# cvlab-stonybrook/s-volsdf

Hardware: AMD Instinct MI355X
Metric: rendered rays/sec (1024-ray batch, 128 samples) (higher is better)
Workload: dtype f32 (every product, forward and backward, as three fp16 MFMA products of two-piece fp16 operands with f32 accumulate; activation blocks hold both pieces: float32 accuracy class); 1 GPU; configs[1]: VolOpt.train_step (forward + MVS prior lookup + loss + backward + clip/guard/Adam), train mode, fast=1: 1024 rays/GPU x 128 coarse + 98 composited samples + 2048 eikonal points, 8x256 SDF MLP + 4x256 radiance MLP; mode=train, mlp_precision=fp16x2, launch=eager launches, rays_per_gpu=1024, rays_total=1024

## Files before the change

s-volsdf_amd/csrc/svs_wgrad.hip:

```cpp
#include "svs_common.h"
#include "svs_mlp_layout.h"
#include "svs_ticket.h"
#include <cstdlib>

namespace svs {
namespace wgrad {

struct Pair {
  const float* a;
  const float* b;
  size_t stride_a, stride_b;
};

struct Args {
  Pair p[2];
  int n_pairs;
  int n_tiles;
  int n_valid_points;
  const float* b_extra;
  size_t stride_extra;
  float* dW;
  int ldw;
  float* db;
  det::Ticket ticket;
};

struct Staging {
  f32x4 a[8], b[8], x;
};

template <int NTB>
__global__ __launch_bounds__(256, 1) void wgrad_kernel(Args a) {
  constexpr int PA = 260, PB = NTB == 9 ? 292 : 260;
  constexpr int BUF = 32 * (PA + PB);
  extern __shared__ __attribute__((aligned(16))) float smem[];
  const int tid = threadIdx.x, wave = tid >> 6, lane = tid & 63;
  const int half = lane >> 5, col = lane & 31;
  f32x16 acc[2][NTB];
#pragma unroll
  for (int o = 0; o < 2; ++o)
#pragma unroll
    for (int i = 0; i < NTB; ++i) acc[o][i] = (f32x16)(0.0f);
  float bias_acc = 0.0f;

  const int my_tiles = a.n_tiles > (int)blockIdx.x ? (a.n_tiles - 1 - (int)blockIdx.x) / (int)gridDim.x + 1 : 0;
  const int n_items = my_tiles * a.n_pairs;
  Staging st;
  int st_live = 32;

  auto issue = [&](int item) {
    const int t = blockIdx.x + (item / a.n_pairs) * gridDim.x, pi = item % a.n_pairs;
    const Pair& p = a.p[pi];
    const f32x4* ga = reinterpret_cast<const f32x4*>(p.a + (size_t)t * p.stride_a);
    const f32x4* gb = reinterpret_cast<const f32x4*>(p.b + (size_t)t * p.stride_b);
#pragma unroll
    for (int k = 0; k < 8; ++k) { st.a[k] = ga[k * 256 + tid]; st.b[k] = gb[k * 256 + tid]; }
    if (NTB == 9) {
      st.x = (a.b_extra && pi == 0) ? reinterpret_cast<const f32x4*>(a.b_extra + (size_t)t * a.stride_extra)[tid]
                                    : (f32x4)(0.0f);
    }
    st_live = a.n_valid_points - t * 32;
  };
  auto commit = [&](int buf) {
    float* la = smem + buf * BUF;
    float* lb = la + 32 * PA;
    if (st_live < 32) {
#pragma unroll
      for (int k = 0; k < 8; ++k) if ((tid & 31) >= st_live) st.a[k] = (f32x4)(0.0f);
    }
#pragma unroll
    for (int k = 0; k < 8; ++k) {
      const int q = k * 256 + tid, i4 = q >> 6, ln = q & 63;
      const int feat = 32 * (i4 >> 2) + 8 * (i4 & 3) + 4 * (ln >> 5), pt = ln & 31;
      *reinterpret_cast<f32x4*>(la + pt * PA + feat) = st.a[k];
      *reinterpret_cast<f32x4*>(lb + pt * PB + feat) = st.b[k];
    }
    if (NTB == 9) {
      const int i4 = tid >> 6, ln = tid & 63;
      *reinterpret_cast<f32x4*>(lb + (ln & 31) * PB + 256 + 8 * i4 + 4 * (ln >> 5)) = st.x;
    }
  };

  if (n_items > 0) { issue(0); commit(0); }
  __syncthreads();
  for (int item = 0; item < n_items; ++item) {
    const int buf = item & 1;
    const bool more = item + 1 < n_items;
    if (more) issue(item + 1);
    const float* la = smem + buf * BUF;
    const float* lb = la + 32 * PA;
    if (a.db && (item % a.n_pairs) == 0) {
      float s = 0.0f;
#pragma unroll 8
      for (int q = 0; q < 32; ++q) s += la[q * PA + tid];
      bias_acc += s;
    }
#pragma unroll 4
    for (int s = 0; s < 16; ++s) {
      const int pt = 2 * s + half;
      const float a0 = la[pt * PA + 32 * (2 * wave) + col];
      const float a1 = la[pt * PA + 32 * (2 * wave + 1) + col];
#pragma unroll
      for (int i = 0; i < NTB; ++i) {
        const float b = lb[pt * PB + 32 * i + col];
        acc[0][i] = __builtin_amdgcn_mfma_f32_32x32x2f32(a0, b, acc[0][i], 0, 0, 0);
        acc[1][i] = __builtin_amdgcn_mfma_f32_32x32x2f32(a1, b, acc[1][i], 0, 0, 0);
      }
    }
    if (more) commit(buf ^ 1);
    __syncthreads();
  }
  det::wait_turn(a.ticket, blockIdx.x);
#pragma unroll
  for (int o = 0; o < 2; ++o)
#pragma unroll
    for (int i = 0; i < NTB; ++i)
#pragma unroll
      for (int r = 0; r < 16; ++r) {
        const int row = 32 * (2 * wave + o) + rho(r) + 4 * half;
        const int c = 32 * i + col;
        if (c < a.ldw) atomicAdd(&a.dW[(size_t)row * a.ldw + c], acc[o][i][r]);
      }
  if (a.db) atomicAdd(&a.db[tid], bias_acc);
  det::pass_turn(a.ticket, blockIdx.x);
}


namespace h2 {

typedef _Float16 f16x8 __attribute__((ext_vector_type(8)));
typedef _Float16 f16x4 __attribute__((ext_vector_type(4)));
typedef _Float16 f16x2 __attribute__((ext_vector_type(2)));
typedef short s16x4 __attribute__((__vector_size__(4 * sizeof(short))));
#define SVS_LDS(T, ptr) ((__attribute__((address_space(3))) T*)(ptr))

constexpr int kPlane = 16384;
constexpr int kExtraPiece = 32 * 64;
constexpr int kNarrowImg = 8192;
constexpr int kRecBytes = 8 * 256;
constexpr int kFactorBytes = 8 * 64;
template <bool GP>
struct Ring {
  static constexpr int kPlanes = GP ? 2 : 1;
  static constexpr int kSlot = 2 * kPlanes * kPlane;
  static constexpr int kB = kPlanes * kPlane;
  static constexpr int kRing = GP ? 2 : 4;
  static constexpr int kAhead = kRing - 1;
  static constexpr int kSlotAll = kSlot + kRecBytes + kFactorBytes;
  static constexpr int kLdsBytes = kRing * kSlotAll;
};

struct Frag { s16x4 lo, hi; };
__device__ __forceinline__ void tr_issue(Frag& v, unsigned a0, unsigned a1) {
  asm volatile("ds_read_b64_tr_b16 %0, %1" : "=v"(v.lo) : "v"(a0));
  asm volatile("ds_read_b64_tr_b16 %0, %1" : "=v"(v.hi) : "v"(a1));
}
__device__ __forceinline__ f16x8 frag_of(const Frag& v) { return __builtin_bit_cast(f16x8, v); }
__device__ __forceinline__ void lds_read128(f32x4& v, unsigned a) { asm volatile("ds_read_b128 %0, %1" : "=v"(v) : "v"(a)); }
__device__ __forceinline__ void lds_read32(float& v, unsigned a) { asm volatile("ds_read_b32 %0, %1" : "=v"(v) : "v"(a)); }
__device__ __forceinline__ void lds_wait() {
  asm volatile("s_waitcnt lgkmcnt(0)" ::: "memory");
  __builtin_amdgcn_sched_barrier(0);
}
__device__ __forceinline__ unsigned lds_addr(const void* p) {
  return (unsigned)(unsigned long long)SVS_LDS(const void, p);
}

__device__ __forceinline__ void scale_from_absmax(const float* absmax, float& s, float& inv_s) {
  s = 1.0f; inv_s = 1.0f;
  if (!absmax) return;
  int e = (int)((__float_as_uint(*absmax) >> 23) & 0xff);
  e = e < 16 ? 16 : (e > 250 ? 250 : e);
  s = __uint_as_float((unsigned)(268 - e) << 23);
  inv_s = __uint_as_float((unsigned)(e - 14) << 23);
}

struct Job {
  Pair p[2];
  const float* rec[2];
  int n_pairs;
  int n_tiles;
  int n_valid_points;
  int b_tiles;
  int col0;
  float* dW;
  int ldw;
  float* db;
  const float* absmax;
  int wg_begin, wg_count;
  det::Ticket ticket;
};
constexpr int kMaxJobs = 20;
struct MultiArgs { Job job[kMaxJobs]; int n_jobs; int touch; int reverse; };
static_assert(sizeof(MultiArgs) <= 4096, "kernel arguments");

constexpr int kThreadsW = 512;

typedef const __attribute__((address_space(1))) void* gvoid;

template <bool GP>
__global__ __launch_bounds__(kThreadsW, 1) void wgrad_h2_multi_kernel(MultiArgs ma) {
  typedef Ring<GP> R;
  constexpr int kSlot = R::kSlot, kSlotAll = R::kSlotAll, kRing = R::kRing, kAhead = R::kAhead, kB = R::kB;
  extern __shared__ __attribute__((aligned(16))) unsigned char smem_h2[];
  int jj = 0;
  for (int q = 1; q < ma.n_jobs; ++q) if ((int)blockIdx.x >= ma.job[q].wg_begin) jj = q;
  const Job& a = ma.job[jj];
  const int wg = (int)blockIdx.x - a.wg_begin, nwg = a.wg_count;
  const int tid = threadIdx.x, lane = tid & 63;
  const int wave = __builtin_amdgcn_readfirstlane(tid >> 6);
  const bool narrow = a.b_tiles == 1;
  float s_grad, inv_s;
  scale_from_absmax(a.absmax, s_grad, inv_s);

  f32x16 acc[8];
#pragma unroll
  for (int i = 0; i < 8; ++i) acc[i] = (f32x16)(0.0f);
  float bsum = 0.0f;

  unsigned char* ring = smem_h2;

  const int rq = (lane & 15) >> 2, rp = lane & 3, rg = (lane >> 4) & 1, rh = lane >> 5;
  const int rd0 = 1024 * rg + 256 * rh + 128 * rg + 64 * (rp & 1) + 16 * rq + 8 * (rp >> 1);
  const int a_rd = 2048 * wave + rd0;
  const int rx0 = 64 * (8 * rh + rq) + 32 * rg + 8 * rp, rx1 = rx0 + 64 * 4;
  const int wp = lane & 31, whf = lane >> 5;
  const int wxoff = 64 * wp + 16 * (wave & 3) + 8 * whf;

  const bool two_pairs = a.n_pairs == 2;
  const int my_tiles = a.n_tiles > wg ? (a.n_tiles - 1 - wg) / nwg + 1 : 0;
  const int n_items = two_pairs ? 2 * my_tiles : my_tiles;
  const int n_valid = a.n_valid_points;
  const bool has_db = a.db != nullptr;
  const bool rev = ma.reverse != 0;
  const float* const pa0 = a.p[0].a; const float* const pb0 = a.p[0].b;
  const float* const pa1 = a.p[1].a; const float* const pb1 = a.p[1].b;
  const size_t sa0 = a.p[0].stride_a, sb0 = a.p[0].stride_b, sa1 = a.p[1].stride_a, sb1 = a.p[1].stride_b;
  const float* const rec0 = a.rec[0]; const float* const rec1 = a.rec[1];
  const bool has_scale = a.absmax != nullptr;
  auto tile_of = [&](int item) {
    const int k = two_pairs ? item >> 1 : item;
    return rev ? wg + (my_tiles - 1 - k) * nwg : wg + k * nwg;
  };

  auto issue = [&](int item) {
    const int t = tile_of(item), pi = two_pairs ? item & 1 : 0;
    const float* pa = (pi ? pa1 : pa0) + (size_t)t * (pi ? sa1 : sa0);
    const float* pb = (pi ? pb1 : pb0) + (size_t)t * (pi ? sb1 : sb0);
    unsigned char* slot = ring + (item % kRing) * kSlotAll;
#pragma unroll
    for (int j = 0; j < 2 * R::kPlanes; ++j) {
      const int piece = wave + 8 * j;
      __builtin_amdgcn_global_load_lds((gvoid)(reinterpret_cast<const f32x4*>(pa) + piece * 64 + lane),
                                       SVS_LDS(void, slot + piece * 1024), 16, 0, 0);
      if (!narrow)
        __builtin_amdgcn_global_load_lds((gvoid)(reinterpret_cast<const f32x4*>(pb) + piece * 64 + lane),
                                         SVS_LDS(void, slot + kB + piece * 1024), 16, 0, 0);
    }
    if (narrow)
      __builtin_amdgcn_global_load_lds((gvoid)(reinterpret_cast<const f32x4*>(pb) + (wave & 3) * 64 + lane),
                                       SVS_LDS(void, slot + kB + (wave & 3) * 1024), 16, 0, 0);
    if (has_scale)
      __builtin_amdgcn_global_load_lds((gvoid)((pi ? rec1 : rec0) + (size_t)t * 64 + lane),
                                       SVS_LDS(void, slot + kSlot + wave * 256), 4, 0, 0);
  };
  unsigned sink = 0;
  auto touch = [&](int item) {
    const int t = tile_of(item), pi = two_pairs ? item & 1 : 0;
    const Pair& p = a.p[pi];
    constexpr int kLines = R::kPlanes * (kPlane / 128);
    const int nb = narrow ? 32 : kLines;
    const float* q = tid < kLines ? p.a + (size_t)t * p.stride_a + tid * 32
                                  : p.b + (size_t)t * p.stride_b + (tid - kLines) * 32;
    if (tid < kLines + nb) asm volatile("global_load_dword %0, %1, off" : "+v"(sink) : "v"(q) : "memory");
  };
  const int ops = (narrow ? 2 * R::kPlanes + 1 : 4 * R::kPlanes) + (has_scale ? 1 : 0);

  auto stage_factors = [&](int item) {
    unsigned char* slot = ring + (item % kRing) * kSlotAll;
    const int t = tile_of(item);
    const int live = n_valid - t * 32;
    float f = 1.0f;
    if (has_scale) {
      float rec;
      lds_read32(rec, lds_addr(slot + kSlot + wave * 256 + 4 * wp));
      lds_wait();
      const unsigned eb = (__float_as_uint(rec) >> 23) & 0xff;
      if (eb >= 20 && eb <= 240) f = __builtin_fminf(s_grad * __uint_as_float((254u << 23) - __float_as_uint(rec)), 32768.0f);
    }
    if (wp >= live) f = 0.0f;
    if (lane < 32) asm volatile("ds_write_b16 %0, %1" :: "v"(lds_addr(slot + kSlot + kRecBytes + wave * 64 + 2 * lane)), "v"((_Float16)f) : "memory");
  };
  auto stage_narrow = [&](int item) {
    unsigned char* slot = ring + (item % kRing) * kSlotAll;
    if (tid < 256) {
      f32x4 v;
      lds_read128(v, lds_addr(slot + kB + tid * 16));
      lds_wait();
      f16x4 hi, mid;
#pragma unroll
      for (int j = 0; j < 4; ++j) {
        const _Float16 h = (_Float16)v[j];
        hi[j] = h;
        mid[j] = (_Float16)(v[j] - (float)h);
      }
      *SVS_LDS(f16x4, slot + kB + kNarrowImg + wxoff) = hi;
      *SVS_LDS(f16x4, slot + kB + kNarrowImg + kExtraPiece + wxoff) = mid;
    }
  };

  const f16x2 one2 = {(_Float16)1.0f, (_Float16)1.0f};

  for (int i0 = 0; i0 < kAhead && i0 < n_items; ++i0) issue(i0);
  const bool touching = GP && ma.touch;
  bool touched = false;
  if (touching && kAhead < n_items) { touch(kAhead); touched = true; }
  auto pre_stage = [&](int it) {
    const int left = n_items - 1 - it;
    const int later = (left < kAhead - 1 ? left : kAhead - 1) * ops;
    if (later == 10) asm volatile("s_waitcnt vmcnt(10)" ::: "memory");
    else if (later == 8) asm volatile("s_waitcnt vmcnt(8)" ::: "memory");
    else if (later == 6) asm volatile("s_waitcnt vmcnt(6)" ::: "memory");
    else if (later == 5) asm volatile("s_waitcnt vmcnt(5)" ::: "memory");
    else if (later == 4) asm volatile("s_waitcnt vmcnt(4)" ::: "memory");
    else if (later == 3) asm volatile("s_waitcnt vmcnt(3)" ::: "memory");
    else if (touched) asm volatile("s_waitcnt vmcnt(1)" ::: "memory");
    else asm volatile("s_waitcnt vmcnt(0)" ::: "memory");
    stage_factors(it);
  };
  for (int item = 0; item < n_items; ++item) {
    const int pi = two_pairs ? item & 1 : 0;
    const bool p0 = pi == 0;
    pre_stage(item);
    asm volatile("s_waitcnt lgkmcnt(0)\n\ts_barrier" ::: "memory");
    if (narrow) {
      stage_narrow(item);
      asm volatile("s_waitcnt lgkmcnt(0)\n\ts_barrier" ::: "memory");
    }
    auto issue_next = [&]() {
      if (item + kAhead < n_items) issue(item + kAhead);
      touched = false;
      if (touching && item + kAhead + 1 < n_items) { touch(item + kAhead + 1); touched = true; }
    };
    const unsigned la = lds_addr(ring + (item % kRing) * kSlotAll);
    const unsigned lb = la + kB;
    const unsigned ftab = la + kSlot + kRecBytes + wave * 64;
    const unsigned nimg = lb + kNarrowImg;
    const bool want_bias = has_db && p0;
    const bool two = narrow;
    Frag fa2[2], fam2[2];
    f32x4 fraw2[2];
#pragma unroll
    for (int ks = 0; ks < 2; ++ks) {
      tr_issue(fa2[ks], la + 512 * ks + a_rd, la + 512 * ks + (a_rd ^ 128));
      if (GP) tr_issue(fam2[ks], la + kPlane + 512 * ks + a_rd, la + kPlane + 512 * ks + (a_rd ^ 128));
      lds_read128(fraw2[ks], ftab + 32 * ks + 16 * rh);
    }
    issue_next();
    lds_wait();
#pragma unroll
    for (int ks = 0; ks < 2; ++ks) {
      const f16x8 ah = frag_of(fa2[ks]) * __builtin_bit_cast(f16x8, fraw2[ks]);
      const f16x8 am = GP ? frag_of(fam2[ks]) * __builtin_bit_cast(f16x8, fraw2[ks]) : ah;
      if (want_bias) {
#pragma unroll
        for (int j = 0; j < 4; ++j) {
          const f16x2 h2v = {ah[2 * j], ah[2 * j + 1]};
          bsum = __builtin_amdgcn_fdot2(h2v, one2, bsum, false);
          if (GP) {
            const f16x2 m2v = {am[2 * j], am[2 * j + 1]};
            bsum = __builtin_amdgcn_fdot2(m2v, one2, bsum, false);
          }
        }
      }
#pragma unroll
      for (int i = 0; i < 8; ++i) {
        if (i > 0 && narrow) break;
        Frag fh, fm;
        if (!narrow) {
          const unsigned rd = lb + 2048 * i + 512 * ks + rd0;
          tr_issue(fh, rd, rd ^ 128);
          if (GP) tr_issue(fm, rd + kPlane, (rd ^ 128) + kPlane);
        } else {
          tr_issue(fh, nimg + ks * 1024 + rx0, nimg + ks * 1024 + rx1);
          tr_issue(fm, nimg + kExtraPiece + ks * 1024 + rx0, nimg + kExtraPiece + ks * 1024 + rx1);
        }
        lds_wait();
        if (two || GP) acc[i] = __builtin_amdgcn_mfma_f32_32x32x16_f16(ah, frag_of(fm), acc[i], 0, 0, 0);
        if (GP) acc[i] = __builtin_amdgcn_mfma_f32_32x32x16_f16(am, frag_of(fh), acc[i], 0, 0, 0);
        acc[i] = __builtin_amdgcn_mfma_f32_32x32x16_f16(ah, frag_of(fh), acc[i], 0, 0, 0);
      }
    }
  }
  asm volatile("s_waitcnt vmcnt(0)" :: "v"(sink) : "memory");
  const int half = lane >> 5, col = lane & 31;
  det::wait_turn(a.ticket, wg);
#pragma unroll
  for (int i = 0; i < 8; ++i) {
    if (i > 0 && narrow) break;
#pragma unroll
    for (int r = 0; r < 16; ++r) {
      const int row = 32 * wave + rho(r) + 4 * half;
      const int c = a.col0 + 32 * i + col;
      if (c < a.ldw) atomicAdd(&a.dW[(size_t)row * a.ldw + c], acc[i][r] * inv_s);
    }
  }
  if (a.db) {
    bsum += __shfl_xor(bsum, 32);
    if (half == 0) atomicAdd(&a.db[32 * wave + col], bsum * inv_s);
  }
  det::pass_turn(a.ticket, wg);
}

}

}
}

using namespace svs;
using namespace svs::wgrad;
namespace h2 = svs::wgrad::h2;

extern "C" {

struct svs_wgrad_job {
  const float *a0, *b0; long long sa0, sb0;
  const float *a1, *b1; long long sa1, sb1;
  const float* b_extra; long long s_extra;
  int n_points, ldw;
  float *dW, *db;
  const float* absmax;
  const float *rec0, *rec1;
};

int svs_wgrad_multi(const svs_wgrad_job* jobs, int n_jobs, int precision, void* hip_stream) {
  if (!jobs || n_jobs < 1) { set_error("svs_wgrad_multi: no jobs"); return SVS_EINVAL; }
  int n_expanded = 0;
  for (int j = 0; j < n_jobs; ++j) n_expanded += jobs[j].b_extra ? 2 : 1;
  if (n_expanded > h2::kMaxJobs) { set_error("svs_wgrad_multi: at most %d jobs (b_extra counts twice)", h2::kMaxJobs); return SVS_EINVAL; }
  for (int j = 0; j < n_jobs; ++j) {
    const svs_wgrad_job& q = jobs[j];
    if (!q.a0 || !q.b0 || !q.dW || q.n_points <= 0 || q.ldw < 256 || q.ldw > 288 || (q.b_extra && q.ldw < 288) || (q.a1 && !q.b1)) {
      set_error("svs_wgrad_multi: bad argument in job %d", j); return SVS_EINVAL;
    }
    if (mlp::is_h2(precision) && q.absmax && (!q.rec0 || (q.a1 && !q.rec1))) {
      set_error("svs_wgrad_multi: job %d has absmax but no scale records", j); return SVS_EINVAL;
    }
  }
  hipStream_t s = (hipStream_t)hip_stream;
  if (mlp::is_h2(precision)) {
    const bool gp = precision == mlp::kFmtF16x2;
    h2::MultiArgs ma;
    int n = 0;
    long long work[h2::kMaxJobs], total = 0;
    for (int j = 0; j < n_jobs; ++j) {
      const svs_wgrad_job& q = jobs[j];
      h2::Job& J = ma.job[n];
      J.p[0] = Pair{q.a0, q.b0, (size_t)q.sa0, (size_t)q.sb0};
      J.rec[0] = q.rec0; J.rec[1] = q.rec1;
      J.n_pairs = 1;
      if (q.a1) { J.p[1] = Pair{q.a1, q.b1, (size_t)q.sa1, (size_t)q.sb1}; J.n_pairs = 2; }
      else { J.p[1] = J.p[0]; J.rec[1] = J.rec[0]; }
      J.n_tiles = (q.n_points + 31) / 32; J.n_valid_points = q.n_points;
      J.b_tiles = 8; J.col0 = 0; J.dW = q.dW; J.ldw = q.ldw; J.db = q.db; J.absmax = q.absmax;
      work[n] = (long long)J.n_tiles * J.n_pairs * 10;
      total += work[n++];
      if (q.b_extra) {
        h2::Job& X = ma.job[n];
        X = J;
        X.p[0].b = q.b_extra; X.p[0].stride_b = (size_t)q.s_extra; X.n_pairs = 1;
        X.b_tiles = 1; X.col0 = 256; X.db = nullptr;
        work[n] = (long long)X.n_tiles * 6;
        total += work[n++];
      }
    }
    ma.n_jobs = n;
    static const int touch_env = [] { const char* e = getenv("SVS_WGRAD_TOUCH"); return e ? atoi(e) : 0; }();
    ma.touch = touch_env;
    static const int reverse_env = [] { const char* e = getenv("SVS_WGRAD_REVERSE"); return e ? atoi(e) : 0; }();
    ma.reverse = reverse_env;
    (void)total;
    const int n_wg_total = 256;
    int count[h2::kMaxJobs];
    int used = 0;
    for (int j = 0; j < n; ++j) { count[j] = 1; ++used; }
    while (used < n_wg_total) {
      int best = -1;
      double load = 0.0;
      for (int j = 0; j < n; ++j) {
        if (count[j] >= ma.job[j].n_tiles) continue;
        const double l = (double)work[j] / count[j];
        if (l > load) { load = l; best = j; }
      }
      if (best < 0) break;
      ++count[best]; ++used;
    }
    int begin = 0;
    for (int j = 0; j < n; ++j) {
      ma.job[j].wg_begin = begin; ma.job[j].wg_count = count[j];
      begin += count[j];
      ma.job[j].ticket = det::Ticket{nullptr, 0u, 0u};
    }
    if (deterministic()) {
      int owner[h2::kMaxJobs], n_owner = 0;
      for (int j = 0; j < n; ++j) {
        owner[j] = -1;
        for (int k = 0; k < j; ++k)
          if (ma.job[k].dW == ma.job[j].dW && ma.job[k].col0 == ma.job[j].col0) { owner[j] = owner[k]; break; }
        if (owner[j] < 0) owner[j] = n_owner++;
      }
      unsigned* turn = det::take_slots((unsigned)n_owner);
      if (!turn) { set_error("svs_wgrad_multi: no turn counters (deterministic mode)"); return SVS_EINVAL; }
      unsigned total[h2::kMaxJobs] = {0};
      for (int j = 0; j < n; ++j) { ma.job[j].ticket.turn = turn + owner[j]; ma.job[j].ticket.first = total[owner[j]]; total[owner[j]] += (unsigned)count[j]; }
      for (int j = 0; j < n; ++j) ma.job[j].ticket.total = total[owner[j]];
    }
    static hipError_t e = hipFuncSetAttribute(reinterpret_cast<const void*>(h2::wgrad_h2_multi_kernel<false>),
                                              hipFuncAttributeMaxDynamicSharedMemorySize, h2::Ring<false>::kLdsBytes);
    static hipError_t ep = hipFuncSetAttribute(reinterpret_cast<const void*>(h2::wgrad_h2_multi_kernel<true>),
                                               hipFuncAttributeMaxDynamicSharedMemorySize, h2::Ring<true>::kLdsBytes);
    if (e != hipSuccess || ep != hipSuccess) {
      set_error("svs_wgrad_multi: hipFuncSetAttribute: %s", hipGetErrorString(e != hipSuccess ? e : ep)); return (int)(e != hipSuccess ? e : ep);
    }
    if (gp) h2::wgrad_h2_multi_kernel<true><<<begin, h2::kThreadsW, h2::Ring<true>::kLdsBytes, s>>>(ma);
    else h2::wgrad_h2_multi_kernel<false><<<begin, h2::kThreadsW, h2::Ring<false>::kLdsBytes, s>>>(ma);
    return check_launch("svs_wgrad_multi");
  }
  if (precision != mlp::kFmtF32) { set_error("svs_wgrad_multi: unknown precision %d", precision); return SVS_EINVAL; }
  for (int j = 0; j < n_jobs; ++j) {
    const svs_wgrad_job& q = jobs[j];
    Args a;
    a.p[0] = Pair{q.a0, q.b0, (size_t)q.sa0, (size_t)q.sb0};
    a.n_pairs = 1;
    if (q.a1) { a.p[1] = Pair{q.a1, q.b1, (size_t)q.sa1, (size_t)q.sb1}; a.n_pairs = 2; }
    a.n_tiles = (q.n_points + 31) / 32;
    a.n_valid_points = q.n_points;
    a.b_extra = q.b_extra; a.stride_extra = (size_t)q.s_extra;
    a.dW = q.dW; a.ldw = q.ldw; a.db = q.db;
    const int grid = a.n_tiles < 256 ? a.n_tiles : 256;
    a.ticket = det::Ticket{det::take_slots(1), 0u, (unsigned)grid};
    if (q.b_extra) {
      constexpr int lds = 2 * 32 * (260 + 292) * 4;
      static hipError_t e9 = hipFuncSetAttribute(reinterpret_cast<const void*>(wgrad_kernel<9>),
                                                 hipFuncAttributeMaxDynamicSharedMemorySize, lds);
      if (e9 != hipSuccess) { set_error("svs_wgrad_multi: hipFuncSetAttribute: %s", hipGetErrorString(e9)); return (int)e9; }
      wgrad_kernel<9><<<grid, 256, lds, s>>>(a);
    } else {
      constexpr int lds = 2 * 32 * (260 + 260) * 4;
      static hipError_t e8 = hipFuncSetAttribute(reinterpret_cast<const void*>(wgrad_kernel<8>),
                                                 hipFuncAttributeMaxDynamicSharedMemorySize, lds);
      if (e8 != hipSuccess) { set_error("svs_wgrad_multi: hipFuncSetAttribute: %s", hipGetErrorString(e8)); return (int)e8; }
      wgrad_kernel<8><<<grid, 256, lds, s>>>(a);
    }
    if (int rc = check_launch("svs_wgrad_multi")) return rc;
  }
  return SVS_OK;
}

int svs_wgrad(const float* a0, const float* b0, long long sa0, long long sb0, const float* a1, const float* b1,
              long long sa1, long long sb1, const float* b_extra, long long s_extra, int n_points, int precision,
              const float* absmax, const float* rec0, const float* rec1, float* dW, int ldw, float* db, void* hip_stream) {
  svs_wgrad_job q{a0, b0, sa0, sb0, a1, b1, sa1, sb1, b_extra, s_extra, n_points, ldw, dW, db, absmax, rec0, rec1};
  return svs_wgrad_multi(&q, 1, precision, hip_stream);
}

}
```

Before: 290,600 rays/s.

## Fold extra-input weight-gradient columns into the main wgrad job

```diff
diff --git a/s-volsdf_amd/csrc/svs_wgrad.hip b/s-volsdf_amd/csrc/svs_wgrad.hip
--- a/s-volsdf_amd/csrc/svs_wgrad.hip
+++ b/s-volsdf_amd/csrc/svs_wgrad.hip
@@ -136,7 +136,7 @@
 
 constexpr int kPlane = 16384;
 constexpr int kExtraPiece = 32 * 64;
-constexpr int kNarrowImg = 8192;
+constexpr int kExtraBytes = 4096;
 constexpr int kRecBytes = 8 * 256;
 constexpr int kFactorBytes = 8 * 64;
 template <bool GP>
@@ -147,8 +147,11 @@
   static constexpr int kRing = GP ? 2 : 4;
   static constexpr int kAhead = kRing - 1;
   static constexpr int kSlotAll = kSlot + kRecBytes + kFactorBytes;
-  static constexpr int kLdsBytes = kRing * kSlotAll;
+  static constexpr int kXRaw = kRing * kSlotAll;
+  static constexpr int kXImg = kXRaw + kAhead * kExtraBytes;
+  static constexpr int kLdsBytes = kXImg + 2 * kExtraBytes;
 };
+static_assert(Ring<true>::kLdsBytes <= 160 * 1024 && Ring<false>::kLdsBytes <= 160 * 1024, "LDS of a CU");
 
 struct Frag { s16x4 lo, hi; };
 __device__ __forceinline__ void tr_issue(Frag& v, unsigned a0, unsigned a1) {
@@ -181,8 +184,8 @@
   int n_pairs;
   int n_tiles;
   int n_valid_points;
-  int b_tiles;
-  int col0;
+  const float* x;
+  size_t stride_x;
   float* dW;
   int ldw;
   float* db;
@@ -209,13 +212,12 @@
   const int wg = (int)blockIdx.x - a.wg_begin, nwg = a.wg_count;
   const int tid = threadIdx.x, lane = tid & 63;
   const int wave = __builtin_amdgcn_readfirstlane(tid >> 6);
-  const bool narrow = a.b_tiles == 1;
   float s_grad, inv_s;
   scale_from_absmax(a.absmax, s_grad, inv_s);
 
-  f32x16 acc[8];
-#pragma unroll
-  for (int i = 0; i < 8; ++i) acc[i] = (f32x16)(0.0f);
+  f32x16 acc[9];
+#pragma unroll
+  for (int i = 0; i < 9; ++i) acc[i] = (f32x16)(0.0f);
   float bsum = 0.0f;
 
   unsigned char* ring = smem_h2;
@@ -238,6 +240,11 @@
   const size_t sa0 = a.p[0].stride_a, sb0 = a.p[0].stride_b, sa1 = a.p[1].stride_a, sb1 = a.p[1].stride_b;
   const float* const rec0 = a.rec[0]; const float* const rec1 = a.rec[1];
   const bool has_scale = a.absmax != nullptr;
+  const float* const px = a.x;
+  const size_t sx = a.stride_x;
+  const bool has_x = px != nullptr;
+  const bool x_wave = has_x && wave < 4;
+  const unsigned xraw = lds_addr(ring + R::kXRaw), ximg = lds_addr(ring + R::kXImg);
   auto tile_of = [&](int item) {
     const int k = two_pairs ? item >> 1 : item;
     return rev ? wg + (my_tiles - 1 - k) * nwg : wg + k * nwg;
@@ -253,13 +260,12 @@
       const int piece = wave + 8 * j;
       __builtin_amdgcn_global_load_lds((gvoid)(reinterpret_cast<const f32x4*>(pa) + piece * 64 + lane),
                                        SVS_LDS(void, slot + piece * 1024), 16, 0, 0);
-      if (!narrow)
-        __builtin_amdgcn_global_load_lds((gvoid)(reinterpret_cast<const f32x4*>(pb) + piece * 64 + lane),
-                                         SVS_LDS(void, slot + kB + piece * 1024), 16, 0, 0);
-    }
-    if (narrow)
-      __builtin_amdgcn_global_load_lds((gvoid)(reinterpret_cast<const f32x4*>(pb) + (wave & 3) * 64 + lane),
-                                       SVS_LDS(void, slot + kB + (wave & 3) * 1024), 16, 0, 0);
+      __builtin_amdgcn_global_load_lds((gvoid)(reinterpret_cast<const f32x4*>(pb) + piece * 64 + lane),
+                                       SVS_LDS(void, slot + kB + piece * 1024), 16, 0, 0);
+    }
+    if (x_wave)
+      __builtin_amdgcn_global_load_lds((gvoid)(reinterpret_cast<const f32x4*>(px + (size_t)t * sx) + wave * 64 + lane),
+                                       SVS_LDS(void, ring + R::kXRaw + (item % kAhead) * kExtraBytes + wave * 1024), 16, 0, 0);
     if (has_scale)
       __builtin_amdgcn_global_load_lds((gvoid)((pi ? rec1 : rec0) + (size_t)t * 64 + lane),
                                        SVS_LDS(void, slot + kSlot + wave * 256), 4, 0, 0);
@@ -269,12 +275,11 @@
     const int t = tile_of(item), pi = two_pairs ? item & 1 : 0;
     const Pair& p = a.p[pi];
     constexpr int kLines = R::kPlanes * (kPlane / 128);
-    const int nb = narrow ? 32 : kLines;
     const float* q = tid < kLines ? p.a + (size_t)t * p.stride_a + tid * 32
                                   : p.b + (size_t)t * p.stride_b + (tid - kLines) * 32;
-    if (tid < kLines + nb) asm volatile("global_load_dword %0, %1, off" : "+v"(sink) : "v"(q) : "memory");
-  };
-  const int ops = (narrow ? 2 * R::kPlanes + 1 : 4 * R::kPlanes) + (has_scale ? 1 : 0);
+    if (tid < 2 * kLines) asm volatile("global_load_dword %0, %1, off" : "+v"(sink) : "v"(q) : "memory");
+  };
+  const int ops = 4 * R::kPlanes + (has_scale ? 1 : 0) + (x_wave ? 1 : 0);
 
   auto stage_factors = [&](int item) {
     unsigned char* slot = ring + (item % kRing) * kSlotAll;
@@ -291,22 +296,20 @@
     if (wp >= live) f = 0.0f;
     if (lane < 32) asm volatile("ds_write_b16 %0, %1" :: "v"(lds_addr(slot + kSlot + kRecBytes + wave * 64 + 2 * lane)), "v"((_Float16)f) : "memory");
   };
-  auto stage_narrow = [&](int item) {
-    unsigned char* slot = ring + (item % kRing) * kSlotAll;
-    if (tid < 256) {
-      f32x4 v;
-      lds_read128(v, lds_addr(slot + kB + tid * 16));
-      lds_wait();
-      f16x4 hi, mid;
-#pragma unroll
-      for (int j = 0; j < 4; ++j) {
-        const _Float16 h = (_Float16)v[j];
-        hi[j] = h;
-        mid[j] = (_Float16)(v[j] - (float)h);
-      }
-      *SVS_LDS(f16x4, slot + kB + kNarrowImg + wxoff) = hi;
-      *SVS_LDS(f16x4, slot + kB + kNarrowImg + kExtraPiece + wxoff) = mid;
-    }
+  auto stage_extras = [&](int item) {
+    f32x4 v;
+    lds_read128(v, xraw + (item % kAhead) * kExtraBytes + tid * 16);
+    lds_wait();
+    f16x4 hi, mid;
+#pragma unroll
+    for (int j = 0; j < 4; ++j) {
+      const _Float16 h = (_Float16)v[j];
+      hi[j] = h;
+      mid[j] = (_Float16)(v[j] - (float)h);
+    }
+    const unsigned img = ximg + (item & 1) * kExtraBytes + wxoff;
+    asm volatile("ds_write_b64 %0, %1" :: "v"(img), "v"(hi) : "memory");
+    asm volatile("ds_write_b64 %0, %1" :: "v"(img + kExtraPiece), "v"(mid) : "memory");
   };
 
   const f16x2 one2 = {(_Float16)1.0f, (_Float16)1.0f};
@@ -318,25 +321,22 @@
   auto pre_stage = [&](int it) {
     const int left = n_items - 1 - it;
     const int later = (left < kAhead - 1 ? left : kAhead - 1) * ops;
-    if (later == 10) asm volatile("s_waitcnt vmcnt(10)" ::: "memory");
+    if (later == 12) asm volatile("s_waitcnt vmcnt(12)" ::: "memory");
+    else if (later == 10) asm volatile("s_waitcnt vmcnt(10)" ::: "memory");
     else if (later == 8) asm volatile("s_waitcnt vmcnt(8)" ::: "memory");
     else if (later == 6) asm volatile("s_waitcnt vmcnt(6)" ::: "memory");
     else if (later == 5) asm volatile("s_waitcnt vmcnt(5)" ::: "memory");
     else if (later == 4) asm volatile("s_waitcnt vmcnt(4)" ::: "memory");
-    else if (later == 3) asm volatile("s_waitcnt vmcnt(3)" ::: "memory");
     else if (touched) asm volatile("s_waitcnt vmcnt(1)" ::: "memory");
     else asm volatile("s_waitcnt vmcnt(0)" ::: "memory");
     stage_factors(it);
+    if (x_wave && !(two_pairs && (it & 1))) stage_extras(it);
   };
   for (int item = 0; item < n_items; ++item) {
     const int pi = two_pairs ? item & 1 : 0;
     const bool p0 = pi == 0;
     pre_stage(item);
     asm volatile("s_waitcnt lgkmcnt(0)\n\ts_barrier" ::: "memory");
-    if (narrow) {
-      stage_narrow(item);
-      asm volatile("s_waitcnt lgkmcnt(0)\n\ts_barrier" ::: "memory");
-    }
     auto issue_next = [&]() {
       if (item + kAhead < n_items) issue(item + kAhead);
       touched = false;
@@ -345,9 +345,9 @@
     const unsigned la = lds_addr(ring + (item % kRing) * kSlotAll);
     const unsigned lb = la + kB;
     const unsigned ftab = la + kSlot + kRecBytes + wave * 64;
-    const unsigned nimg = lb + kNarrowImg;
+    const unsigned nimg = ximg + (item & 1) * kExtraBytes;
     const bool want_bias = has_db && p0;
-    const bool two = narrow;
+    const bool want_x = has_x && p0;
     Frag fa2[2], fam2[2];
     f32x4 fraw2[2];
 #pragma unroll
@@ -375,20 +375,23 @@
       }
 #pragma unroll
       for (int i = 0; i < 8; ++i) {
-        if (i > 0 && narrow) break;
         Frag fh, fm;
-        if (!narrow) {
-          const unsigned rd = lb + 2048 * i + 512 * ks + rd0;
-          tr_issue(fh, rd, rd ^ 128);
-          if (GP) tr_issue(fm, rd + kPlane, (rd ^ 128) + kPlane);
-        } else {
-          tr_issue(fh, nimg + ks * 1024 + rx0, nimg + ks * 1024 + rx1);
-          tr_issue(fm, nimg + kExtraPiece + ks * 1024 + rx0, nimg + kExtraPiece + ks * 1024 + rx1);
-        }
+        const unsigned rd = lb + 2048 * i + 512 * ks + rd0;
+        tr_issue(fh, rd, rd ^ 128);
+        if (GP) tr_issue(fm, rd + kPlane, (rd ^ 128) + kPlane);
         lds_wait();
-        if (two || GP) acc[i] = __builtin_amdgcn_mfma_f32_32x32x16_f16(ah, frag_of(fm), acc[i], 0, 0, 0);
+        if (GP) acc[i] = __builtin_amdgcn_mfma_f32_32x32x16_f16(ah, frag_of(fm), acc[i], 0, 0, 0);
         if (GP) acc[i] = __builtin_amdgcn_mfma_f32_32x32x16_f16(am, frag_of(fh), acc[i], 0, 0, 0);
         acc[i] = __builtin_amdgcn_mfma_f32_32x32x16_f16(ah, frag_of(fh), acc[i], 0, 0, 0);
+      }
+      if (want_x) {
+        Frag fh, fm;
+        tr_issue(fh, nimg + ks * 1024 + rx0, nimg + ks * 1024 + rx1);
+        tr_issue(fm, nimg + kExtraPiece + ks * 1024 + rx0, nimg + kExtraPiece + ks * 1024 + rx1);
+        lds_wait();
+        acc[8] = __builtin_amdgcn_mfma_f32_32x32x16_f16(ah, frag_of(fm), acc[8], 0, 0, 0);
+        if (GP) acc[8] = __builtin_amdgcn_mfma_f32_32x32x16_f16(am, frag_of(fh), acc[8], 0, 0, 0);
+        acc[8] = __builtin_amdgcn_mfma_f32_32x32x16_f16(ah, frag_of(fh), acc[8], 0, 0, 0);
       }
     }
   }
@@ -396,13 +399,14 @@
   const int half = lane >> 5, col = lane & 31;
   det::wait_turn(a.ticket, wg);
 #pragma unroll
-  for (int i = 0; i < 8; ++i) {
-    if (i > 0 && narrow) break;
-#pragma unroll
-    for (int r = 0; r < 16; ++r) {
-      const int row = 32 * wave + rho(r) + 4 * half;
-      const int c = a.col0 + 32 * i + col;
-      if (c < a.ldw) atomicAdd(&a.dW[(size_t)row * a.ldw + c], acc[i][r] * inv_s);
+  for (int i = 0; i < 9; ++i) {
+    if (i < 8 || has_x) {
+#pragma unroll
+      for (int r = 0; r < 16; ++r) {
+        const int row = 32 * wave + rho(r) + 4 * half;
+        const int c = 32 * i + col;
+        if (c < a.ldw) atomicAdd(&a.dW[(size_t)row * a.ldw + c], acc[i][r] * inv_s);
+      }
     }
   }
   if (a.db) {
@@ -435,9 +439,7 @@
 
 int svs_wgrad_multi(const svs_wgrad_job* jobs, int n_jobs, int precision, void* hip_stream) {
   if (!jobs || n_jobs < 1) { set_error("svs_wgrad_multi: no jobs"); return SVS_EINVAL; }
-  int n_expanded = 0;
-  for (int j = 0; j < n_jobs; ++j) n_expanded += jobs[j].b_extra ? 2 : 1;
-  if (n_expanded > h2::kMaxJobs) { set_error("svs_wgrad_multi: at most %d jobs (b_extra counts twice)", h2::kMaxJobs); return SVS_EINVAL; }
+  if (n_jobs > h2::kMaxJobs) { set_error("svs_wgrad_multi: at most %d jobs", h2::kMaxJobs); return SVS_EINVAL; }
   for (int j = 0; j < n_jobs; ++j) {
     const svs_wgrad_job& q = jobs[j];
     if (!q.a0 || !q.b0 || !q.dW || q.n_points <= 0 || q.ldw < 256 || q.ldw > 288 || (q.b_extra && q.ldw < 288) || (q.a1 && !q.b1)) {
@@ -462,17 +464,10 @@
       if (q.a1) { J.p[1] = Pair{q.a1, q.b1, (size_t)q.sa1, (size_t)q.sb1}; J.n_pairs = 2; }
       else { J.p[1] = J.p[0]; J.rec[1] = J.rec[0]; }
       J.n_tiles = (q.n_points + 31) / 32; J.n_valid_points = q.n_points;
-      J.b_tiles = 8; J.col0 = 0; J.dW = q.dW; J.ldw = q.ldw; J.db = q.db; J.absmax = q.absmax;
-      work[n] = (long long)J.n_tiles * J.n_pairs * 10;
+      J.x = q.b_extra; J.stride_x = (size_t)q.s_extra;
+      J.dW = q.dW; J.ldw = q.ldw; J.db = q.db; J.absmax = q.absmax;
+      work[n] = (long long)J.n_tiles * (J.n_pairs * 10 + (q.b_extra ? 1 : 0));
       total += work[n++];
-      if (q.b_extra) {
-        h2::Job& X = ma.job[n];
-        X = J;
-        X.p[0].b = q.b_extra; X.p[0].stride_b = (size_t)q.s_extra; X.n_pairs = 1;
-        X.b_tiles = 1; X.col0 = 256; X.db = nullptr;
-        work[n] = (long long)X.n_tiles * 6;
-        total += work[n++];
-      }
     }
     ma.n_jobs = n;
     static const int touch_env = [] { const char* e = getenv("SVS_WGRAD_TOUCH"); return e ? atoi(e) : 0; }();
@@ -506,7 +501,7 @@
       for (int j = 0; j < n; ++j) {
         owner[j] = -1;
         for (int k = 0; k < j; ++k)
-          if (ma.job[k].dW == ma.job[j].dW && ma.job[k].col0 == ma.job[j].col0) { owner[j] = owner[k]; break; }
+          if (ma.job[k].dW == ma.job[j].dW) { owner[j] = owner[k]; break; }
         if (owner[j] < 0) owner[j] = n_owner++;
       }
       unsigned* turn = det::take_slots((unsigned)n_owner);
```

Result: no change. 292,600 rays/s, median of 6 (+0.7%).
